# alibaba/unified-audio

Hardware: NVIDIA H100
Metric: hcodec2_encode_rvq_decode_samples_per_s (higher is better)
Workload: dtype f16x3/f16 tensor-core, f32 accumulate

## Files before the change

### unified_audio_b200/csrc/lstm_tc.cu

```cuda
#include <atomic>
#include <cstdio>
#include <cstdlib>

#include "common.cuh"
#include "quark_b200.h"
#include "wgmma.cuh"

namespace qb {
extern std::atomic<long long> g_launches;

constexpr int LT_GROUPS = 4, LT_THREADS = LT_GROUPS * 128 + 32;
constexpr int LT_KG = 4;
constexpr int LT_STAGES = 4;
constexpr uint32_t LT_KBLK = 32 * 128;
constexpr uint32_t LT_SLOT = LT_KBLK * LT_KG;
constexpr uint32_t LT_PAD = 4 * 1024;

__device__ __forceinline__ unsigned lt_ld_relaxed(const unsigned* p) {
  unsigned v;
  asm volatile("ld.relaxed.gpu.global.u32 %0, [%1];" : "=r"(v) : "l"(p) : "memory");
  return v;
}
__device__ __forceinline__ void bulk_load_1d(void* smem_dst, const void* gsrc, uint32_t bytes, uint64_t* bar) {
  asm volatile("cp.async.bulk.shared::cluster.global.mbarrier::complete_tx::bytes [%0], [%1], %2, [%3];"
               ::"r"(smem_u32(smem_dst)), "l"(gsrc), "r"(bytes), "r"(smem_u32(bar)) : "memory");
}

__device__ __forceinline__ float lt_rcp(float x) {
  float r;
  asm("rcp.approx.ftz.f32 %0, %1;" : "=f"(r) : "f"(x));
  return r;
}
__device__ __forceinline__ float lt_sigmoid(float x) { return lt_rcp(1.0f + __expf(-x)); }
__device__ __forceinline__ float lt_tanh(float x) { return fmaf(-2.0f, lt_rcp(1.0f + __expf(2.0f * x)), 1.0f); }

template <int U>
__global__ void __launch_bounds__(LT_THREADS, 1)
lstm_tc_kernel(const __grid_constant__ CUtensorMap tmW,
               const float* __restrict__ xp, int B, int T, int H, __half* __restrict__ out_hi,
               __half* __restrict__ out_lo, __half* hbuf, unsigned* flags, int n_groups, int poll_ns) {
  constexpr int N = 4 * U;
  constexpr int UPT = N / 8;
  static_assert(N % 16 == 0 && N <= 48, "unsupported slice width");
  constexpr uint32_t WBLK = N * 128;
  extern __shared__ uint8_t smem_raw[];
  uint8_t* smem = (uint8_t*)(((uintptr_t)smem_raw + 1023) & ~(uintptr_t)1023);
  const int KB = H / 64, SLOTS = KB / LT_KG;
  uint8_t* Wsm = smem;
  uint8_t* ring = smem + (size_t)KB * WBLK;
  uint64_t* full = (uint64_t*)(ring + LT_STAGES * LT_SLOT + LT_PAD);
  uint64_t* empty = full + LT_STAGES;
  uint64_t* wbar = empty + LT_STAGES;
  int* slot_tag = (int*)(wbar + 1);

  const int tid = threadIdx.x, warp = tid >> 5, lane = tid & 31;
  const int u0 = blockIdx.x * U, G = gridDim.x;

  if (tid == 0) {
    for (int s = 0; s < LT_STAGES; ++s) { mbar_init(&full[s], 1); mbar_init(&empty[s], 4); }
    mbar_init(wbar, 1);
    for (int s = 0; s < LT_STAGES; ++s) slot_tag[s] = -1;
    fence_mbar_init();
  }
  for (int i = tid; i < (int)((LT_STAGES * LT_SLOT + LT_PAD) / 16); i += LT_THREADS)
    reinterpret_cast<uint4*>(ring)[i] = make_uint4(0, 0, 0, 0);
  fence_proxy_async();
  __syncthreads();

  if (warp == LT_GROUPS * 4) {
    if (lane == 0) {
      prefetch_tmap(&tmW);
      mbar_arrive_expect_tx(wbar, (uint32_t)KB * WBLK);
      for (int kb = 0; kb < KB; ++kb) tma_load_2d(Wsm + (size_t)kb * WBLK, &tmW, wbar, kb * 64, blockIdx.x * N);
    }
    uint32_t stage = 0, phase = 0;
    int slot = 0;
    for (int t = 1; t < T; ++t) {
      for (int g = 0; g < n_groups; ++g) {
        const unsigned* fl = flags + (size_t)g * G;
        unsigned spins = 0;
        for (;;) {
          bool ok = true;
          for (int c = lane; c < G; c += 32) ok = ok && (lt_ld_relaxed(fl + c) >= (unsigned)t);
          if (__all_sync(0xffffffffu, ok)) break;
          if (poll_ns) __nanosleep(poll_ns);
          if (++spins > (1u << 24)) asm volatile("trap;");
        }
        asm volatile("fence.acq_rel.gpu;" ::: "memory");
        __syncwarp();
        if (lane == 0) {
          asm volatile("fence.proxy.async;" ::: "memory");
          const int buf = (t + 1) & 1;
          for (int kb = 0; kb < KB; kb += LT_KG, ++slot) {
            mbar_wait(&empty[stage], phase ^ 1);
            mbar_arrive_expect_tx(&full[stage], LT_SLOT);
            __threadfence_block();
            *(volatile int*)(slot_tag + stage) = slot;
            bulk_load_1d(ring + stage * LT_SLOT, hbuf + (((size_t)buf * n_groups + g) * KB + kb) * (LT_KBLK / 2), LT_SLOT,
                         &full[stage]);
            if (++stage == LT_STAGES) { stage = 0; phase ^= 1; }
          }
        }
        __syncwarp();
      }
    }
  } else {
    const int g = warp >> 2, wq = warp & 3;
    if (g < n_groups) {
      const int rr = wq * 16 + (lane >> 2) + (lane & 1) * 8;
      const int n = g * 32 + rr;
      const bool act = wq < 2 && n < B;
      float c[UPT];
#pragma unroll
      for (int i = 0; i < UPT; ++i) c[i] = 0.f;
      mbar_wait(wbar, 0);
      for (int t = 0; t < T; ++t) {
        __half* hcur = hbuf + ((size_t)(t & 1) * n_groups + g) * KB * (LT_KBLK / 2);
        float xg[4][UPT];
#pragma unroll
        for (int gg = 0; gg < 4; ++gg)
#pragma unroll
          for (int j = 0; j < UPT; ++j)
            xg[gg][j] = act ? xp[((long long)n * T + t) * 4 * H + (long long)gg * H + u0 + 2 * j + ((lane >> 1) & 1)] : 0.f;
        float acc[N / 2];
#pragma unroll
        for (int i = 0; i < N / 2; ++i) acc[i] = 0.f;
        if (t > 0) {
          const long long s0 = ((long long)(t - 1) * n_groups + g) * SLOTS;
          for (int sidx = 0; sidx < SLOTS; ++sidx) {
            const long long q = s0 + sidx;
            const int stage = (int)(q % LT_STAGES);
            unsigned spins = 0;
            while (*(volatile int*)(slot_tag + stage) != (int)q)
              if (++spins > (1u << 26)) asm volatile("trap;");
            __threadfence_block();
            mbar_wait(&full[stage], (uint32_t)((q / LT_STAGES) & 1));
            wgmma_fence();
#pragma unroll
            for (int j = 0; j < LT_KG; ++j) {
              const int kb = sidx * LT_KG + j;
              const uint32_t sa = smem_u32(ring + stage * LT_SLOT + j * LT_KBLK), sw = smem_u32(Wsm + (size_t)kb * WBLK);
#pragma unroll
              for (int k = 0; k < 4; ++k)
                Wgmma<N>::ss(acc, make_wgmma_desc_sw128(sa + k * 32), make_wgmma_desc_sw128(sw + k * 32), 1u);
            }
            wgmma_commit();
            wgmma_wait<0>();
            wgmma_fence_regs(acc);
            if (lane == 0) mbar_arrive(&empty[stage]);
          }
        }
        if (wq < 2) {
          const bool odd = lane & 1;
#pragma unroll
          for (int j = 0; j < UPT; ++j) {
            const float s0 = odd ? acc[4 * j] : acc[4 * j + 2], s1 = odd ? acc[4 * j + 1] : acc[4 * j + 3];
            const float r0 = __shfl_xor_sync(0xffffffffu, s0, 1), r1 = __shfl_xor_sync(0xffffffffu, s1, 1);
            const float a_i = odd ? r0 : acc[4 * j], a_f = odd ? r1 : acc[4 * j + 1];
            const float a_g = odd ? acc[4 * j + 2] : r0, a_o = odd ? acc[4 * j + 3] : r1;
            if (act) {
              const float ig = lt_sigmoid(a_i + xg[0][j]), fg = lt_sigmoid(a_f + xg[1][j]);
              const float cg = lt_tanh(a_g + xg[2][j]), og = lt_sigmoid(a_o + xg[3][j]);
              const float cn = fg * c[j] + ig * cg;
              c[j] = cn;
              __half hv, lv;
              split_f16(og * lt_tanh(cn), hv, lv);
              const int uu = u0 + 2 * j + ((lane >> 1) & 1), kbk = uu >> 6, col = uu & 63;
              hcur[kbk * (int)(LT_KBLK / 2) + rr * 64 + ((((col >> 3) ^ (rr & 7)) << 3) | (col & 7))] = hv;
              const long long o = ((long long)n * T + t) * H + uu;
              out_hi[o] = hv;
              if (out_lo) out_lo[o] = lv;
            }
          }
          asm volatile("bar.sync %0, 64;" ::"r"(1 + g) : "memory");
          if (wq == 0 && lane == 0) {
            asm volatile("st.release.gpu.global.u32 [%0], %1;" ::"l"(flags + (size_t)g * G + blockIdx.x), "r"((unsigned)(t + 1))
                         : "memory");
          }
        }
      }
    }
  }
}

typedef CUresult (*EncodeTiledFn)(CUtensorMap*, CUtensorMapDataType, cuuint32_t, void*, const cuuint64_t*,
                                  const cuuint64_t*, const cuuint32_t*, const cuuint32_t*, CUtensorMapInterleave,
                                  CUtensorMapSwizzle, CUtensorMapL2promotion, CUtensorMapFloatOOBfill);
static EncodeTiledFn lt_encode() {
  static EncodeTiledFn fn = nullptr;
  if (!fn) {
    void* p = nullptr;
    cudaDriverEntryPointQueryResult q;
    if (cudaGetDriverEntryPoint("cuTensorMapEncodeTiled", &p, cudaEnableDefault, &q) == cudaSuccess &&
        q == cudaDriverEntryPointSuccess)
      fn = (EncodeTiledFn)p;
  }
  return fn;
}

static int lstm_tc_chunk(const float* xp, const qb_half* whh_perm, int U, int B, int64_t T, int64_t H, __half* oh, __half* ol,
                         void* workspace, cudaStream_t st) {
  const int N = 4 * U, grid = (int)(H / U), KB = (int)(H / 64);
  const int n_groups = (B + 31) / 32, Bp = n_groups * 32;
  EncodeTiledFn enc = lt_encode();
  QB_REQUIRE(enc != nullptr, "cuTensorMapEncodeTiled not available");
  CUtensorMap tmW;
  {
    cuuint64_t dims[2] = {(cuuint64_t)H, (cuuint64_t)(4 * H)};
    cuuint64_t str[1] = {(cuuint64_t)H * 2};
    cuuint32_t box[2] = {64, (cuuint32_t)N};
    cuuint32_t es[2] = {1, 1};
    CUresult r = enc(&tmW, CU_TENSOR_MAP_DATA_TYPE_FLOAT16, 2, (void*)whh_perm, dims, str, box, es, CU_TENSOR_MAP_INTERLEAVE_NONE,
                     CU_TENSOR_MAP_SWIZZLE_128B, CU_TENSOR_MAP_L2_PROMOTION_L2_256B, CU_TENSOR_MAP_FLOAT_OOB_FILL_NONE);
    QB_REQUIRE(r == CUDA_SUCCESS, "lstm_tc: W tensor map failed (%d)", (int)r);
  }
  __half* hbuf = (__half*)workspace;
  const size_t smem = (size_t)KB * N * 128 + (size_t)LT_STAGES * LT_SLOT + LT_PAD + 1024 + 256;
  QB_REQUIRE(smem <= 227 * 1024, "lstm_tc: shared memory budget exceeded (%zu)", smem);
  const size_t hbytes = (size_t)2 * Bp * H * 2;
  QB_CHECK_CUDA(cudaMemsetAsync(workspace, 0, hbytes + 4096, st));
  unsigned* flags = (unsigned*)((uint8_t*)workspace + hbytes);
  int Bi = B, Ti = (int)T, Hi = (int)H, ng = n_groups;
  static int poll_ns = -1;
  if (poll_ns < 0) { const char* e = getenv("QB_LSTM_POLL_NS"); poll_ns = e ? atoi(e) : 0; }
  void* args[] = {&tmW, &xp, &Bi, &Ti, &Hi, &oh, &ol, &hbuf, &flags, &ng, &poll_ns};
  const void* fn = U == 4 ? (const void*)lstm_tc_kernel<4> : U == 8 ? (const void*)lstm_tc_kernel<8> : (const void*)lstm_tc_kernel<12>;
  QB_CHECK_CUDA(cudaFuncSetAttribute(fn, cudaFuncAttributeMaxDynamicSharedMemorySize, (int)smem));
  QB_CHECK_CUDA(cudaLaunchCooperativeKernel(fn, dim3(grid), dim3(LT_THREADS), args, smem, st));
  g_launches++;
  return 0;
}

}
using namespace qb;

extern "C" int32_t qb_lstm_tc_units(int64_t H) {
  int dev = 0, sms = 0;
  if (cudaGetDevice(&dev) != cudaSuccess || cudaDeviceGetAttribute(&sms, cudaDevAttrMultiProcessorCount, dev) != cudaSuccess)
    sms = 132;
  for (int U : {4, 8, 12}) if (H % U == 0 && H / U <= sms) return U;
  return 0;
}

extern "C" int64_t qb_lstm_tc_workspace_bytes(int64_t B, int64_t H) {
  const int64_t Bc = B < 128 ? B : 128;
  const int64_t Bp = ceil_div(Bc, 32) * 32;
  return 2 * Bp * H * 2 + 4096;
}

extern "C" int qb_lstm_tc(const float* xp, const qb_half* whh_perm, int32_t units, int64_t B, int64_t T, int64_t H,
                          qb_half* out_hi, qb_half* out_lo, void* workspace, void* stream) {
  cudaStream_t st = (cudaStream_t)stream;
  QB_REQUIRE(xp && whh_perm && out_hi && workspace, "lstm_tc: bad args");
  QB_REQUIRE(H % (64 * LT_KG) == 0 && (units == 4 || units == 8 || units == 12) && H % units == 0, "lstm_tc: unsupported H / units");
  QB_REQUIRE(B >= 1, "lstm_tc: empty batch");
  for (int64_t b0 = 0; b0 < B; b0 += 128) {
    const int bc = (int)(B - b0 < 128 ? B - b0 : 128);
    if (int e = lstm_tc_chunk(xp + b0 * T * 4 * H, whh_perm, units, bc, T, H, (__half*)out_hi + b0 * T * H,
                              out_lo ? (__half*)out_lo + b0 * T * H : nullptr, workspace, st))
      return e;
  }
  return 0;
}
```

Before: 142.2 million.

## Vectorize LSTM flag polling with acquire loads and overlap wgmma slot waits

```diff
diff --git a/unified_audio_b200/csrc/lstm_tc.cu b/unified_audio_b200/csrc/lstm_tc.cu
--- a/unified_audio_b200/csrc/lstm_tc.cu
+++ b/unified_audio_b200/csrc/lstm_tc.cu
@@ -1,6 +1,5 @@
 #include <atomic>
 #include <cstdio>
-#include <cstdlib>
 
 #include "common.cuh"
 #include "quark_b200.h"
@@ -16,9 +15,9 @@
 constexpr uint32_t LT_SLOT = LT_KBLK * LT_KG;
 constexpr uint32_t LT_PAD = 4 * 1024;
 
-__device__ __forceinline__ unsigned lt_ld_relaxed(const unsigned* p) {
-  unsigned v;
-  asm volatile("ld.relaxed.gpu.global.u32 %0, [%1];" : "=r"(v) : "l"(p) : "memory");
+__device__ __forceinline__ uint4 lt_ld_acquire4(const unsigned* p) {
+  uint4 v;
+  asm volatile("ld.acquire.gpu.global.v4.u32 {%0, %1, %2, %3}, [%4];" : "=r"(v.x), "=r"(v.y), "=r"(v.z), "=r"(v.w) : "l"(p) : "memory");
   return v;
 }
 __device__ __forceinline__ void bulk_load_1d(void* smem_dst, const void* gsrc, uint32_t bytes, uint64_t* bar) {
@@ -38,7 +37,7 @@
 __global__ void __launch_bounds__(LT_THREADS, 1)
 lstm_tc_kernel(const __grid_constant__ CUtensorMap tmW,
                const float* __restrict__ xp, int B, int T, int H, __half* __restrict__ out_hi,
-               __half* __restrict__ out_lo, __half* hbuf, unsigned* flags, int n_groups, int poll_ns) {
+               __half* __restrict__ out_lo, __half* hbuf, unsigned* flags, int n_groups) {
   constexpr int N = 4 * U;
   constexpr int UPT = N / 8;
   static_assert(N % 16 == 0 && N <= 48, "unsupported slice width");
@@ -81,12 +80,13 @@
         unsigned spins = 0;
         for (;;) {
           bool ok = true;
-          for (int c = lane; c < G; c += 32) ok = ok && (lt_ld_relaxed(fl + c) >= (unsigned)t);
+          for (int c = 4 * lane; c < G; c += 128) {
+            const uint4 v = lt_ld_acquire4(fl + c);
+            ok = ok && v.x >= (unsigned)t && v.y >= (unsigned)t && v.z >= (unsigned)t && v.w >= (unsigned)t;
+          }
           if (__all_sync(0xffffffffu, ok)) break;
-          if (poll_ns) __nanosleep(poll_ns);
           if (++spins > (1u << 24)) asm volatile("trap;");
         }
-        asm volatile("fence.acq_rel.gpu;" ::: "memory");
         __syncwarp();
         if (lane == 0) {
           asm volatile("fence.proxy.async;" ::: "memory");
@@ -127,6 +127,7 @@
         for (int i = 0; i < N / 2; ++i) acc[i] = 0.f;
         if (t > 0) {
           const long long s0 = ((long long)(t - 1) * n_groups + g) * SLOTS;
+          int prev = 0;
           for (int sidx = 0; sidx < SLOTS; ++sidx) {
             const long long q = s0 + sidx;
             const int stage = (int)(q % LT_STAGES);
@@ -145,13 +146,19 @@
                 Wgmma<N>::ss(acc, make_wgmma_desc_sw128(sa + k * 32), make_wgmma_desc_sw128(sw + k * 32), 1u);
             }
             wgmma_commit();
-            wgmma_wait<0>();
-            wgmma_fence_regs(acc);
-            if (lane == 0) mbar_arrive(&empty[stage]);
-          }
+            if (sidx > 0) {
+              wgmma_wait<1>();
+              if (lane == 0) mbar_arrive(&empty[prev]);
+            }
+            prev = stage;
+          }
+          wgmma_wait<0>();
+          wgmma_fence_regs(acc);
+          if (lane == 0) mbar_arrive(&empty[prev]);
         }
         if (wq < 2) {
           const bool odd = lane & 1;
+          __half hs[UPT], ls[UPT];
 #pragma unroll
           for (int j = 0; j < UPT; ++j) {
             const float s0 = odd ? acc[4 * j] : acc[4 * j + 2], s1 = odd ? acc[4 * j + 1] : acc[4 * j + 3];
@@ -163,19 +170,23 @@
               const float cg = lt_tanh(a_g + xg[2][j]), og = lt_sigmoid(a_o + xg[3][j]);
               const float cn = fg * c[j] + ig * cg;
               c[j] = cn;
-              __half hv, lv;
-              split_f16(og * lt_tanh(cn), hv, lv);
+              split_f16(og * lt_tanh(cn), hs[j], ls[j]);
               const int uu = u0 + 2 * j + ((lane >> 1) & 1), kbk = uu >> 6, col = uu & 63;
-              hcur[kbk * (int)(LT_KBLK / 2) + rr * 64 + ((((col >> 3) ^ (rr & 7)) << 3) | (col & 7))] = hv;
-              const long long o = ((long long)n * T + t) * H + uu;
-              out_hi[o] = hv;
-              if (out_lo) out_lo[o] = lv;
+              hcur[kbk * (int)(LT_KBLK / 2) + rr * 64 + ((((col >> 3) ^ (rr & 7)) << 3) | (col & 7))] = hs[j];
             }
           }
           asm volatile("bar.sync %0, 64;" ::"r"(1 + g) : "memory");
           if (wq == 0 && lane == 0) {
             asm volatile("st.release.gpu.global.u32 [%0], %1;" ::"l"(flags + (size_t)g * G + blockIdx.x), "r"((unsigned)(t + 1))
                          : "memory");
+          }
+          if (act) {
+#pragma unroll
+            for (int j = 0; j < UPT; ++j) {
+              const long long o = ((long long)n * T + t) * H + u0 + 2 * j + ((lane >> 1) & 1);
+              out_hi[o] = hs[j];
+              if (out_lo) out_lo[o] = ls[j];
+            }
           }
         }
       }
@@ -221,9 +232,7 @@
   QB_CHECK_CUDA(cudaMemsetAsync(workspace, 0, hbytes + 4096, st));
   unsigned* flags = (unsigned*)((uint8_t*)workspace + hbytes);
   int Bi = B, Ti = (int)T, Hi = (int)H, ng = n_groups;
-  static int poll_ns = -1;
-  if (poll_ns < 0) { const char* e = getenv("QB_LSTM_POLL_NS"); poll_ns = e ? atoi(e) : 0; }
-  void* args[] = {&tmW, &xp, &Bi, &Ti, &Hi, &oh, &ol, &hbuf, &flags, &ng, &poll_ns};
+  void* args[] = {&tmW, &xp, &Bi, &Ti, &Hi, &oh, &ol, &hbuf, &flags, &ng};
   const void* fn = U == 4 ? (const void*)lstm_tc_kernel<4> : U == 8 ? (const void*)lstm_tc_kernel<8> : (const void*)lstm_tc_kernel<12>;
   QB_CHECK_CUDA(cudaFuncSetAttribute(fn, cudaFuncAttributeMaxDynamicSharedMemorySize, (int)smem));
   QB_CHECK_CUDA(cudaLaunchCooperativeKernel(fn, dim3(grid), dim3(LT_THREADS), args, smem, st));
```

After: 143.1 million (median of 6 runs). About the same (+0.6%).
